# jesselasse/MARL-DMFB

Measured on AMD Instinct MI355X. Metric: env-steps/sec (whole node), 10x10 DMFB 4-droplet fov9, higher is better.
Workload: dtype int8 env state/obs + f64 rewards; fp32 Q-net; 1 GPU; DMFB 10x10, drop_num=4, fov=9, 4096 parallel envs per GPU (BASELINE configs[1]); parallelism=dp1: chips sharded per rank, one flat RCCL all-reduce per learn

## Files before the change

### marl_dmfb_amd/csrc/crnn_ops.hip

```cpp
#include <hip/hip_runtime.h>

#include <cstdint>
#include <cstdio>
#include <cstdlib>

#include "../../include/crnn_ops.h"

#define HIP_ABI_TAG "crnn_ops"
#define HIP_ABI_ERR CRNN_ERR_HIP
#include "hip_abi.h"
#include "crnn_mfma.h"
#include "crnn_mfma19.h"
#include "crnn_bwd19.h"

namespace {

constexpr int kBlock = 512;
constexpr int kA1Stride = 52;
constexpr int kDz1Unit = 108;

constexpr int kLdsBudget = 158 * 1024;

template <int OD> struct GeoB {
    static constexpr int DZ2 = 28;
    static constexpr int DZ_ROW = OD * DZ2 + 4;
    static constexpr int ROW_FLOATS = OD * kA1Stride + OD * DZ2 + 4 + 244 + (OD / 2) * kDz1Unit;
    static constexpr int FIXED_FLOATS = OD * OD * 9;
    static constexpr int RBB = ((kLdsBudget / 4 - FIXED_FLOATS) / ROW_FLOATS) < (kBlock / (2 * OD)) ? ((kLdsBudget / 4 - FIXED_FLOATS) / ROW_FLOATS)
                                                                                                   : (kBlock / (2 * OD));
    static constexpr size_t LDS_FLOATS = (size_t)FIXED_FLOATS + (size_t)RBB * ROW_FLOATS + OD * 28;
    static constexpr int UNITS = OD * (OD / 2);
    static constexpr int NA = UNITS >= kBlock ? kBlock : kBlock / 2;
    static constexpr int NB = UNITS - NA;
    static constexpr int XSLICES = NB > 0 ? (kBlock - NA) / NB : 1;
    static_assert(NB >= 0 && (NB == 0 || (NA + NB * XSLICES <= kBlock && XSLICES <= 8)), "dW2 roles");
    static constexpr int ITEMS3 = (OD / 2) * 9;
    static constexpr int RS3 = kBlock / ITEMS3;
    static constexpr int PART = kBlock * 9 + kBlock * 9 + OD + kBlock * 6 + OD;
};

template <int OD>
__global__ __launch_bounds__(kBlock) void k_conv9_bwd(const int8_t *__restrict__ obs, long obs_stride, long rows,
                                                      const float *__restrict__ a2, long a2_stride, const float *__restrict__ g, long g_stride,
                                                      const float *__restrict__ w2, float *__restrict__ part,
                                                      const float *__restrict__ w1, const float *__restrict__ b1) {
    using G = GeoB<OD>;
    extern __shared__ __attribute__((aligned(16))) float lds[];
    float *s_w2 = lds;
    float *s_a1 = s_w2 + OD * OD * 9;
    float *s_dz2 = s_a1 + G::RBB * OD * kA1Stride;
    float *s_in = s_dz2 + G::RBB * G::DZ_ROW;
    float *s_dz1 = s_in + G::RBB * 244;
    float *s_w1 = s_dz1 + G::RBB * (OD / 2) * kDz1Unit;
    const int tid = threadIdx.x;
    for (int i = tid; i < OD * 27; i += kBlock) s_w1[i] = w1[i];
    if (tid < OD) s_w1[OD * 27 + tid] = b1[tid];
    for (int i = tid; i < OD * OD * 9; i += kBlock) {
        const int c2 = i / (OD * 9), rem = i - c2 * OD * 9, c1 = rem / 9, tap = rem - c1 * 9;
        s_w2[(c2 * 9 + tap) * OD + c1] = w2[i];
    }
    float accB2 = 0.0f, accB1 = 0.0f, accB1y = 0.0f;
    float2 accW2[9], accW1[3];
#pragma unroll
    for (int k = 0; k < 9; ++k) accW2[k] = make_float2(0.0f, 0.0f);
#pragma unroll
    for (int k = 0; k < 3; ++k) accW1[k] = make_float2(0.0f, 0.0f);
    const bool pa_full = tid < G::NA;
    const int pa_unit = pa_full ? tid : G::NA + (G::NB > 0 ? (tid - G::NA) % (G::NB > 0 ? G::NB : 1) : 0);
    const int pa_slice = pa_full ? 0 : (G::NB > 0 ? (tid - G::NA) / (G::NB > 0 ? G::NB : 1) : 0);
    const bool pa_on = pa_full || (G::NB > 0 && pa_slice < G::XSLICES);
    const int pa_step = pa_full ? 1 : G::XSLICES;
    const int pa_c2 = pa_unit / (OD / 2), pa_cp = pa_unit - pa_c2 * (OD / 2);
    const int i3 = tid % G::ITEMS3, s3 = tid / G::ITEMS3;
    const bool p3_on = s3 < G::RS3;
    const int cp_3 = i3 / 9, c0_3 = (i3 - cp_3 * 9) / 3, kx_3 = i3 - cp_3 * 9 - c0_3 * 3;

    constexpr int kSplit2 = G::NB > 0 ? 2 : 4, kBase2 = G::NB > 0 ? kBlock / 2 : 0;
    const int q2 = (tid - kBase2) & (kSplit2 - 1), unit2 = tid >= kBase2 ? (tid - kBase2) / kSplit2 : G::RBB * (OD / 2);
    const int r2 = unit2 / (OD / 2), cp2 = unit2 - r2 * (OD / 2);
    const int br = tid / OD, bc = tid - br * OD;

    const long n_blocks = (rows + G::RBB - 1) / G::RBB;
    const long per = (n_blocks + gridDim.x - 1) / gridDim.x;
    const long blk0 = (long)blockIdx.x * per, blk1 = min(n_blocks, blk0 + per);

    typedef float f32x4 __attribute__((ext_vector_type(4)));
    const int lane = tid & 63, wave = tid >> 6, j16 = lane & 15, kq = lane >> 4;
    const int c_nh = (wave >> 1) & 1, c_sub = (wave & 1) + 2 * (wave >> 2), c_ch = c_nh * 16 + j16;
    const bool c_chv = c_ch < OD;
    constexpr int NPD = (G::RBB * OD * 25 + kBlock - 1) / kBlock, NPI = (G::RBB * 243 + kBlock - 1) / kBlock;
    float pfa[NPD], pfg[NPD];
    int pfi[NPI];
#pragma unroll
    for (int u = 0; u < NPD; ++u) { pfa[u] = 0.0f; pfg[u] = 0.0f; }
#pragma unroll
    for (int u = 0; u < NPI; ++u) pfi[u] = 0;
    auto fetch = [&](long b) {
        const long r0 = b * G::RBB;
        const int rvb = b < blk1 ? (int)min((long)G::RBB, rows - r0) : 0;
        if (rvb <= 0) return;
        int t_ = tid;
        asm volatile("" : "+v"(t_));
#pragma unroll
        for (int u = 0; u < NPD; ++u) {
            const int i = min(t_ + u * kBlock, G::RBB * OD * 25 - 1), rr = i / (OD * 25), rem = i - rr * OD * 25;
            const long row = r0 + min(rr, rvb - 1);
            pfa[u] = a2[row * a2_stride + rem];
            pfg[u] = g[row * g_stride + rem];
        }
#pragma unroll
        for (int u = 0; u < NPI; ++u) {
            const int i = min(t_ + u * kBlock, G::RBB * 243 - 1), rr = i / 243, pp = i - rr * 243;
            pfi[u] = obs[(r0 + min(rr, rvb - 1)) * obs_stride + pp];
        }
    };
    fetch(blk0);
    for (long blk = blk0; blk < blk1; ++blk) {
        const long row0 = blk * G::RBB;
        const int rv = (int)min((long)G::RBB, rows - row0);
        __syncthreads();
        int t_ = tid;
        asm volatile("" : "+v"(t_));
#pragma unroll
        for (int u = 0; u < NPD; ++u) {
            const int i = t_ + u * kBlock, rc = i / 25, k = i - rc * 25;
            if (i < G::RBB * OD * 25) s_dz2[(rc / OD) * G::DZ_ROW + (rc % OD) * G::DZ2 + k] = (rc / OD < rv && pfa[u] > 0.0f) ? pfg[u] : 0.0f;
        }
#pragma unroll
        for (int u = 0; u < NPI; ++u) {
            const int i = t_ + u * kBlock, rr = i / 243, pp = i - rr * 243;
            if (i < G::RBB * 243) s_in[rr * 244 + pp] = rr < rv ? (float)pfi[u] : 0.0f;
        }
        __syncthreads();
        int off1[7], goff[3];
        float bw1[7];
        int kq_ = kq, j_ = j16;
        asm volatile("" : "+v"(kq_), "+v"(j_));
#pragma unroll
        for (int s = 0; s < 7; ++s) {
            const int k = 4 * s + kq_, c0 = k / 9, tap = k - c0 * 9;
            off1[s] = k < 27 ? c0 * 81 + (tap / 3) * 9 + tap % 3 : 0;
            const float w = s_w1[(c_chv ? c_ch : 0) * 27 + (k < 27 ? k : 0)];
            bw1[s] = (c_chv && k < 27) ? w : 0.0f;
        }
        const float c_bias = c_chv ? s_w1[OD * 27 + c_ch] : 0.0f;
#pragma unroll
        for (int qt = 0; qt < 3; ++qt) { const int p = qt * 16 + j_; goff[qt] = (p / 7) * 9 + p % 7; }
        for (int rr = c_sub; rr < G::RBB; rr += 4) {
            float cv[3][7];
#pragma unroll
            for (int qt = 0; qt < 3; ++qt)
#pragma unroll
                for (int s = 0; s < 7; ++s) cv[qt][s] = s_in[rr * 244 + goff[qt] + off1[s]];
            f32x4 acc[3];
#pragma unroll
            for (int qt = 0; qt < 3; ++qt) acc[qt] = f32x4{c_bias, c_bias, c_bias, c_bias};
#pragma unroll
            for (int s = 0; s < 7; ++s)
#pragma unroll
                for (int qt = 0; qt < 3; ++qt) acc[qt] = __builtin_amdgcn_mfma_f32_16x16x4f32(cv[qt][s], bw1[s], acc[qt], 0, 0, 0);
            if (c_chv) {
                float *dst = s_a1 + ((rr * (OD / 2) + (c_ch >> 1)) * kA1Stride + kq * 4) * 2 + (c_ch & 1);
#pragma unroll
                for (int qt = 0; qt < 3; ++qt)
#pragma unroll
                    for (int q = 0; q < 4; ++q) dst[(qt * 16 + q) * 2] = fmaxf(acc[qt][q], 0.0f);
            }
        }
        if (c_sub == 0) {
            const int rr = j16 < G::RBB ? j16 : G::RBB - 1;
            f32x4 acc = {c_bias, c_bias, c_bias, c_bias};
#pragma unroll
            for (int s = 0; s < 7; ++s) acc = __builtin_amdgcn_mfma_f32_16x16x4f32(s_in[rr * 244 + 60 + off1[s]], bw1[s], acc, 0, 0, 0);
            if (c_chv) {
#pragma unroll
                for (int q = 0; q < 4; ++q)
                    if (kq * 4 + q < G::RBB) s_a1[(((kq * 4 + q) * (OD / 2) + (c_ch >> 1)) * kA1Stride + 48) * 2 + (c_ch & 1)] = fmaxf(acc[q], 0.0f);
            }
        }
        __syncthreads();
        auto unit_rows = [&](int c2, int cp, int r_begin, int r_step) {
#pragma unroll 1
            for (int rr = r_begin; rr < rv; rr += r_step) {
                float dz[G::DZ2];
                float2 a[kA1Stride];
                const float4 *pd = (const float4 *)__builtin_assume_aligned(s_dz2 + rr * G::DZ_ROW + c2 * G::DZ2, 16);
                const float4 *pa = (const float4 *)__builtin_assume_aligned(s_a1 + (size_t)(rr * (OD / 2) + cp) * 2 * kA1Stride, 16);
#pragma unroll
                for (int j = 0; j < G::DZ2 / 4; ++j) { const float4 t = pd[j]; dz[4 * j] = t.x; dz[4 * j + 1] = t.y; dz[4 * j + 2] = t.z; dz[4 * j + 3] = t.w; }
#pragma unroll
                for (int j = 0; j < kA1Stride / 2; ++j) { const float4 t = pa[j]; a[2 * j] = make_float2(t.x, t.y); a[2 * j + 1] = make_float2(t.z, t.w); }
#pragma unroll
                for (int kx = 0; kx < 3; ++kx)
#pragma unroll
                    for (int ky = 0; ky < 3; ++ky)
#pragma unroll
                        for (int x = 0; x < 5; ++x)
#pragma unroll
                            for (int y = 0; y < 5; ++y) {
                                const float z = dz[x * 5 + y];
                                const float2 v = a[(x + kx) * 7 + y + ky];
                                accW2[kx * 3 + ky].x = fmaf(z, v.x, accW2[kx * 3 + ky].x);
                                accW2[kx * 3 + ky].y = fmaf(z, v.y, accW2[kx * 3 + ky].y);
                            }
            }
        };
        if (tid < G::RBB * OD && br < rv) {
            const float4 *pd = (const float4 *)__builtin_assume_aligned(s_dz2 + br * G::DZ_ROW + bc * G::DZ2, 16);
            float t = 0.0f;
#pragma unroll
            for (int j = 0; j < 6; ++j) { const float4 v = pd[j]; t += (v.x + v.y) + (v.z + v.w); }
            accB2 += t + pd[6].x;
        }
#ifndef CRNN_PROBE_SKIP_P1
        if (pa_on) unit_rows(pa_c2, pa_cp, pa_slice, pa_step);
#endif
#ifndef CRNN_PROBE_SKIP_P2
        const bool p2 = unit2 < G::RBB * (OD / 2) && r2 < rv;
#else
        const bool p2 = false;
#endif
        if (p2) {
            float2 da[49];
#pragma unroll
            for (int k = 0; k < 49; ++k) da[k] = make_float2(0.0f, 0.0f);
            const int cbeg = q2 * (OD / kSplit2), cend = cbeg + OD / kSplit2;
#pragma unroll 1
            for (int c2 = cbeg; c2 < cend; ++c2) {
                float dz[G::DZ2];
                float2 w[9];
                const float4 *pd = (const float4 *)__builtin_assume_aligned(s_dz2 + r2 * G::DZ_ROW + c2 * G::DZ2, 16);
#pragma unroll
                for (int j = 0; j < G::DZ2 / 4; ++j) { const float4 t = pd[j]; dz[4 * j] = t.x; dz[4 * j + 1] = t.y; dz[4 * j + 2] = t.z; dz[4 * j + 3] = t.w; }
#pragma unroll
                for (int k = 0; k < 9; ++k) w[k] = *(const float2 *)(s_w2 + (c2 * 9 + k) * OD + 2 * cp2);
#pragma unroll
                for (int kx = 0; kx < 3; ++kx)
#pragma unroll
                    for (int ky = 0; ky < 3; ++ky)
#pragma unroll
                        for (int x = 0; x < 5; ++x)
#pragma unroll
                            for (int y = 0; y < 5; ++y) {
                                float2 &d = da[(x + kx) * 7 + y + ky];
                                const float z = dz[x * 5 + y];
                                d.x = fmaf(z, w[kx * 3 + ky].x, d.x);
                                d.y = fmaf(z, w[kx * 3 + ky].y, d.y);
                            }
            }
#ifndef CRNN_PROBE_P2_NO_DPP
#pragma unroll
            for (int k = 0; k < 49; ++k) {
                asm volatile("v_add_f32_dpp %0, %0, %0 quad_perm:[1,0,3,2] row_mask:0xf bank_mask:0xf bound_ctrl:1" : "+v"(da[k].x));
                asm volatile("v_add_f32_dpp %0, %0, %0 quad_perm:[1,0,3,2] row_mask:0xf bank_mask:0xf bound_ctrl:1" : "+v"(da[k].y));
            }
            if (kSplit2 == 4) {
                asm volatile("s_nop 1");
#pragma unroll
                for (int k = 0; k < 49; ++k) {
                    asm volatile("v_add_f32_dpp %0, %0, %0 quad_perm:[2,3,0,1] row_mask:0xf bank_mask:0xf bound_ctrl:1" : "+v"(da[k].x));
                    asm volatile("v_add_f32_dpp %0, %0, %0 quad_perm:[2,3,0,1] row_mask:0xf bank_mask:0xf bound_ctrl:1" : "+v"(da[k].y));
                }
            }
#endif
#ifdef CRNN_PROBE_P2_NO_MASK
            if (q2 == 0 && da[0].x == 12345.678f) {
#else
            if (q2 == 0) {
#endif
                const float4 *act = (const float4 *)__builtin_assume_aligned(s_a1 + (size_t)unit2 * 2 * kA1Stride, 16);
                unsigned long long lx = 0, ly = 0;
#pragma unroll
                for (int j = 0; j < 25; ++j) {
                    const float4 a = act[j];
                    lx |= (unsigned long long)((a.x > 0.0f ? 1u : 0u) | (a.z > 0.0f ? 2u : 0u)) << (2 * j);
                    ly |= (unsigned long long)((a.y > 0.0f ? 1u : 0u) | (a.w > 0.0f ? 2u : 0u)) << (2 * j);
                }
                float4 *dst4 = (float4 *)__builtin_assume_aligned(s_dz1 + (size_t)unit2 * kDz1Unit, 16);
                float sx = 0.0f, sy = 0.0f;
#pragma unroll
                for (int j = 0; j < 25; ++j) {
                    float4 o;
                    o.x = (lx >> (2 * j)) & 1 ? da[2 * j].x : 0.0f;
                    o.y = (ly >> (2 * j)) & 1 ? da[2 * j].y : 0.0f;
                    o.z = (2 * j + 1 < 49 && ((lx >> (2 * j + 1)) & 1)) ? da[2 * j + 1 < 49 ? 2 * j + 1 : 0].x : 0.0f;
                    o.w = (2 * j + 1 < 49 && ((ly >> (2 * j + 1)) & 1)) ? da[2 * j + 1 < 49 ? 2 * j + 1 : 0].y : 0.0f;
                    dst4[j] = o;
                    sx += o.x + o.z;
                    sy += o.y + o.w;
                }
                accB1 += sx;
                accB1y += sy;
            }
        }
        __syncthreads();
        fetch(blk + 1);
#ifdef CRNN_PROBE_SKIP_P3
        if (false) {
#else
        if (p3_on) {
#endif
            for (int rr = s3; rr < rv; rr += G::RS3) {
                const float2 *pd = (const float2 *)(s_dz1 + (size_t)(rr * (OD / 2) + cp_3) * kDz1Unit);
                const float *in = s_in + rr * 244 + c0_3 * 81 + kx_3 * 9;
#pragma unroll
                for (int x = 0; x < 7; ++x) {
                    float2 dz[7];
                    float v[9];
#pragma unroll
                    for (int y = 0; y < 7; ++y) dz[y] = pd[x * 7 + y];
#pragma unroll
                    for (int y = 0; y < 9; ++y) v[y] = in[x * 9 + y];
#pragma unroll
                    for (int ky = 0; ky < 3; ++ky)
#pragma unroll
                        for (int y = 0; y < 7; ++y) {
                            typedef float f32x2 __attribute__((ext_vector_type(2)));
                            const f32x2 r = __builtin_elementwise_fma((f32x2){dz[y].x, dz[y].y}, (f32x2){v[y + ky], v[y + ky]},
                                                                      (f32x2){accW1[ky].x, accW1[ky].y});
                            accW1[ky] = make_float2(r.x, r.y);
                        }
                }
            }
        }
    }
    __syncthreads();
    if (tid < G::RBB * OD) s_dz2[OD * 16 + bc * 16 + br] = accB2;
    if (q2 == 0 && unit2 < G::RBB * (OD / 2)) {
        s_dz2[(2 * cp2) * 16 + r2] = accB1;
        s_dz2[(2 * cp2 + 1) * 16 + r2] = accB1y;
    }
    __syncthreads();
    float *pp = part + (size_t)blockIdx.x * G::PART;
#pragma unroll
    for (int k = 0; k < 9; ++k) { pp[tid * 18 + 2 * k] = accW2[k].x; pp[tid * 18 + 2 * k + 1] = accW2[k].y; }
    if (tid < OD) {
        float t = 0.0f;
        for (int k = 0; k < G::RBB; ++k) t += s_dz2[OD * 16 + tid * 16 + k];
        pp[kBlock * 18 + tid] = t;
    }
#pragma unroll
    for (int k = 0; k < 3; ++k) { pp[kBlock * 18 + OD + tid * 6 + k] = accW1[k].x; pp[kBlock * 18 + OD + tid * 6 + 3 + k] = accW1[k].y; }
    if (tid < OD) {
        float t = 0.0f;
        for (int k = 0; k < G::RBB; ++k) t += s_dz2[tid * 16 + k];
        pp[kBlock * 18 + OD + kBlock * 6 + tid] = t;
    }
}

constexpr int kRedY = 16;
template <int OD>
__global__ __launch_bounds__(64 * kRedY) void k_conv9_bwd_reduce(const float *__restrict__ part, int n_part, float *__restrict__ grads) {
    using G = GeoB<OD>;
    __shared__ float s_sum[kRedY][64];
    const int tx = threadIdx.x & 63, ty = threadIdx.x >> 6;
    const int i = blockIdx.x * 64 + tx;
    const int n2 = OD * OD * 9, nb = OD, n1 = OD * 27;
    float acc = 0.0f;
    if (i < n2 + nb + n1 + nb) {
        int off[8], cnt = 0;
        if (i < n2) {
            const int pair = i / 9, tap = i - pair * 9, c2 = pair / OD, c1 = pair - c2 * OD;
            const int unit = c2 * (OD / 2) + (c1 >> 1), comp = 2 * tap + (c1 & 1);
            if (unit < G::NA) off[cnt++] = unit * 18 + comp;
            else
                for (int sl = 0; sl < G::XSLICES && sl < 8; ++sl) off[cnt++] = (G::NA + sl * G::NB + (unit - G::NA)) * 18 + comp;
        } else if (i < n2 + nb) {
            off[cnt++] = kBlock * 18 + (i - n2);
        } else if (i < n2 + nb + n1) {
            const int jx = i - n2 - nb, c1 = jx / 27, r = jx - c1 * 27, ky = r % 3;
            const int item = (c1 >> 1) * 9 + r / 3;
            for (int sl = 0; sl < G::RS3; ++sl) off[cnt++] = kBlock * 18 + OD + (sl * G::ITEMS3 + item) * 6 + (c1 & 1) * 3 + ky;
        } else {
            off[cnt++] = kBlock * 18 + OD + kBlock * 6 + (i - n2 - nb - n1);
        }
        for (int k = 0; k < cnt; ++k) {
            float a0 = 0.0f, a1 = 0.0f;
            int b = ty;
            for (; b + kRedY < n_part; b += 2 * kRedY) { a0 += part[(size_t)b * G::PART + off[k]]; a1 += part[(size_t)(b + kRedY) * G::PART + off[k]]; }
            if (b < n_part) a0 += part[(size_t)b * G::PART + off[k]];
            acc += a0 + a1;
        }
    }
    s_sum[ty][tx] = acc;
    __syncthreads();
    if (ty == 0 && i < n2 + nb + n1 + nb) {
        float t = 0.0f;
#pragma unroll
        for (int k = 0; k < kRedY; ++k) t += s_sum[k][tx];
        grads[i] = t;
    }
}

constexpr int kMlpBlock = 256, kMlpOut = 10, kMlpMaxIn = 18, kMlpMaxParts = 256, kMlpTailLoads = 64;
__device__ unsigned g_mlp_ticket = 0;
__global__ __launch_bounds__(kMlpBlock) void k_mlp_bwd(const int8_t *__restrict__ obs, long obs_stride, int dir_off,
                                                       const int8_t *__restrict__ onehot, int n_actions, long rows,
                                                       const float *__restrict__ x, long x_stride, const float *__restrict__ g, long g_stride,
                                                       int col0, float *part, float *__restrict__ dw, float *__restrict__ db) {
    __shared__ float s_red[kMlpBlock / 64][kMlpOut * (kMlpMaxIn + 1)];
    __shared__ int s_last;
    const int nin = 2 + n_actions, n_part = (int)gridDim.x;
    float acc[kMlpOut][kMlpMaxIn + 1];
#pragma unroll
    for (int o = 0; o < kMlpOut; ++o)
#pragma unroll
        for (int k = 0; k <= kMlpMaxIn; ++k) acc[o][k] = 0.0f;
    for (long r = (long)blockIdx.x * kMlpBlock + threadIdx.x; r < rows; r += (long)gridDim.x * kMlpBlock) {
        float v[kMlpMaxIn];
        v[0] = (float)obs[r * obs_stride + dir_off];
        v[1] = (float)obs[r * obs_stride + dir_off + 1];
#pragma unroll
        for (int k = 0; k < kMlpMaxIn - 2; ++k) v[2 + k] = k < n_actions ? (float)onehot[r * n_actions + k] : 0.0f;
#pragma unroll
        for (int o = 0; o < kMlpOut; ++o) {
            const float gz = x[r * x_stride + col0 + o] > 0.0f ? g[r * g_stride + col0 + o] : 0.0f;
#pragma unroll
            for (int k = 0; k < kMlpMaxIn; ++k)
                if (k < nin) acc[o][k] = fmaf(gz, v[k], acc[o][k]);
            acc[o][kMlpMaxIn] += gz;
        }
    }
    const int lane = threadIdx.x & 63, wave = threadIdx.x >> 6;
#pragma unroll
    for (int o = 0; o < kMlpOut; ++o)
#pragma unroll
        for (int k = 0; k <= kMlpMaxIn; ++k)
            if (k < nin || k == kMlpMaxIn) {
                float t = acc[o][k];
                for (int d = 32; d > 0; d >>= 1) t += __shfl_xor(t, d);
                if (lane == 0) s_red[wave][o * (kMlpMaxIn + 1) + k] = t;
            }
    __syncthreads();
    const int n_out = kMlpOut * (nin + 1);
    for (int i = threadIdx.x; i < n_out; i += kMlpBlock) {
        const int o = i < kMlpOut * nin ? i / nin : i - kMlpOut * nin, k = i < kMlpOut * nin ? i - o * nin : kMlpMaxIn;
        float t = 0.0f;
#pragma unroll
        for (int w = 0; w < kMlpBlock / 64; ++w) t += s_red[w][o * (kMlpMaxIn + 1) + k];
        part[(size_t)i * n_part + blockIdx.x] = t;
    }
    if (!last_workgroup_arrives(&g_mlp_ticket, gridDim.x, &s_last)) return;
    for (int i = threadIdx.x; i < n_out; i += kMlpBlock) {
        const float *p = part + (size_t)i * n_part;
        float t = 0.0f;
        for (int b0 = 0; b0 < n_part; b0 += kMlpTailLoads) {
            float v[kMlpTailLoads];
#pragma unroll
            for (int u = 0; u < kMlpTailLoads; ++u) v[u] = b0 + u < n_part ? partial_load(p + b0 + u) : 0.0f;
#pragma unroll
            for (int u = 0; u < kMlpTailLoads; ++u)
                if (b0 + u < n_part) t += v[u];
        }
        if (i < kMlpOut * nin) dw[i] = t;
        else db[i - kMlpOut * nin] = t;
    }
}

struct LiveRows { const int32_t *chips; const int32_t *n; int rows_per_chip; };

template <int OD, int RBV>
int launch_rb(const int8_t *obs, long obs_stride, long rows, const float *w1, const float *b1, const float *w2, const float *b2,
              float *out, long out_stride, int out_cols, const int8_t *onehot, int n_actions, const float *mlp_w, const float *mlp_b, hipStream_t s,
              LiveRows live = LiveRows{nullptr, nullptr, 1}) {
    using GM = crnn_mfma::GeoM<OD, RBV>;
    const size_t lds = GM::LDS_FLOATS * sizeof(float);
    static LdsLimit lds_limit;
    if (const int rc = lds_limit.raise((const void *)crnn_mfma::k_conv9_mfma<OD, RBV>, lds)) return rc;
    const long n_blocks = (rows + GM::RB - 1) / GM::RB;
    const long resident = 256L * (long)((size_t)160 * 1024 / lds);
    const int grid = (int)(n_blocks < resident ? n_blocks : resident);
    LAUNCH((crnn_mfma::k_conv9_mfma<OD, RBV>), dim3(grid), dim3(crnn_mfma::kBlockM), lds, s, obs, obs_stride, rows, w1, b1, w2, b2,
           out, out_stride, out_cols, onehot, n_actions, mlp_w, mlp_b, live.chips, live.n, live.rows_per_chip);
    return CRNN_OK;
}

template <int OD>
int launch(const int8_t *obs, long obs_stride, long rows, const float *w1, const float *b1, const float *w2, const float *b2,
           float *out, long out_stride, int out_cols, const int8_t *onehot, int n_actions, const float *mlp_w, const float *mlp_b, hipStream_t s,
           LiveRows live = LiveRows{nullptr, nullptr, 1}) {
    return launch_rb<OD, 0>(obs, obs_stride, rows, w1, b1, w2, b2, out, out_stride, out_cols, onehot, n_actions, mlp_w, mlp_b, s, live);
}

template <int OD>
int launch19(const int8_t *obs, long obs_stride, long rows, const float *w1, const float *b1, const float *w3, const float *b3,
             float *out, long out_stride, int out_cols, const int8_t *onehot, int n_actions, const float *mlp_w, const float *mlp_b, hipStream_t s) {
    using GM = crnn_mfma19::Geo<OD>;
    const size_t lds = GM::LDS_FLOATS * sizeof(float);
    static LdsLimit lds_limit;
    if (const int rc = lds_limit.raise((const void *)crnn_mfma19::k_conv19_mfma<OD>, lds)) return rc;
    const long n_blocks = (rows + GM::RB - 1) / GM::RB;
    const int grid = (int)(n_blocks < 256 ? n_blocks : 256);
    LAUNCH((crnn_mfma19::k_conv19_mfma<OD>), dim3(grid), dim3(crnn_mfma19::kBlockM), lds, s, obs, obs_stride, rows, w1, b1, w3,
           b3, out, out_stride, out_cols, onehot, n_actions, mlp_w, mlp_b);
    return CRNN_OK;
}

template <int OD>
int launch_bwd(const int8_t *obs, long obs_stride, long rows, const float *a2, long a2_stride,
               const float *g, long g_stride, const float *w2, float *part, int grid, float *grads, const float *w1, const float *b1,
               hipStream_t s) {
    using G = GeoB<OD>;
    const size_t lds = G::LDS_FLOATS * sizeof(float);
    static LdsLimit lds_limit;
    if (const int rc = lds_limit.raise((const void *)k_conv9_bwd<OD>, lds)) return rc;
    HIP_TRY(launch_status([&] {
        hipLaunchKernelGGL((k_conv9_bwd<OD>), dim3(grid), dim3(kBlock), lds, s, obs, obs_stride, rows, a2, a2_stride, g, g_stride,
                           w2, part, w1, b1);
        const int n_out = OD * OD * 9 + OD + OD * 27 + OD;
        hipLaunchKernelGGL((k_conv9_bwd_reduce<OD>), dim3((n_out + 63) / 64), dim3(64 * kRedY), 0, s, part, grid, grads);
    }));
    return CRNN_OK;
}

template <int OD>
int launch_bwd19(const int8_t *obs, long obs_stride, long rows, const float *a3, long a3_stride, const float *g, long g_stride,
                 const float *w1, const float *b1, const float *w3, const float *b3, float *part, int n_part, float *grads, hipStream_t s) {
    using G = crnn_bwd19::GeoB19<OD>;
    const size_t lds = G::LDS_FLOATS * sizeof(float);
    static LdsLimit lds_limit;
    if (const int rc = lds_limit.raise((const void *)crnn_bwd19::k_conv19_bwd<OD>, lds)) return rc;
    const long n_blocks = (rows + G::RBB - 1) / G::RBB;
    const int grid = (int)(n_blocks < n_part ? n_blocks : n_part);
    HIP_TRY(launch_status([&] {
        hipLaunchKernelGGL((crnn_bwd19::k_conv19_bwd<OD>), dim3(grid), dim3(crnn_bwd19::kBlockB), lds, s, obs, obs_stride, rows, a3, a3_stride, g,
                           g_stride, w1, b1, w3, b3, part);
        hipLaunchKernelGGL((crnn_bwd19::k_conv19_bwd_reduce<OD>), dim3((G::GRADS + 63) / 64), dim3(64 * crnn_bwd19::kRedY19), 0, s, part, grid, grads);
    }));
    return CRNN_OK;
}

}

// ... 104 lines not shown
```

### marl_dmfb_amd/csrc/crnn_mfma.h

```cpp
#pragma once
#include <hip/hip_runtime.h>

#include <cstdint>

namespace crnn_mfma {

typedef float f32x4 __attribute__((ext_vector_type(4)));

constexpr int kBlockM = 512;

#ifdef CRNN_PROBE_TS
__device__ unsigned long long *g_crnn_ts;
#define CRNN_TS(k) do { if (lane == 0 && ts_it == 1 && g_crnn_ts) g_crnn_ts[((size_t)blockIdx.x * 8 + wave) * 16 + (k)] = __builtin_readcyclecounter(); } while (0)
#else
#define CRNN_TS(k) do { } while (0)
#endif

template <int OD, int RBV = 0, int NW = 8> struct GeoM {
    static constexpr int RB = RBV ? RBV : (OD <= 24 ? 16 : 12);
    static constexpr int CS = 53;
#ifdef CRNN_NO_ROWLANE
    static constexpr bool ROWLANE = false;
#else
    static constexpr bool ROWLANE = RB == 16;
// ... 124 lines not shown
#pragma unroll
        for (int i = 0; i < GS; ++i)
#pragma unroll
            for (int n = 0; n < NT; ++n) {
                const int k = (g % GPQ) * GS + i;
                acc[n] = __builtin_amdgcn_mfma_f32_16x16x4f32(v[g & 1][n][i], bw[(g / GPQ) * 12 + k], acc[n], 0, 0, 0);
            }
        __builtin_amdgcn_sched_barrier(0);
    }
#ifdef CRNN_PROBE_NO_EPI
    if (ok && acc[0][0] == 12345.678f) {
#else
    if (ok) {
#endif
#pragma unroll
        for (int n = 0; n < NT; ++n) {
            float *dst = s_out + kq * 4 * G::OUT_STRIDE + col + (n == 0 ? p0 : p1);
#pragma unroll
            for (int q = 0; q < 4; ++q) dst[q * G::OUT_STRIDE] = fmaxf(acc[n][q], 0.0f);
        }
    }
}

template <int OD, int RBV = 0, int NW = 8>
__global__ __launch_bounds__(64 * NW) void k_conv9_mfma(const int8_t *__restrict__ obs, long obs_stride, long rows,
                                                        const float *__restrict__ w1, const float *__restrict__ b1,
                                                        const float *__restrict__ w2, const float *__restrict__ b2,
                                                        float *__restrict__ out, long out_stride, int out_cols,
                                                        const int8_t *__restrict__ onehot, int n_actions,
                                                        const float *__restrict__ mlp_w, const float *__restrict__ mlp_b,
                                                        const int32_t *__restrict__ live_chips, const int32_t *__restrict__ n_live,
                                                        int rows_per_chip) {
    using G = GeoM<OD, RBV, NW>;
    constexpr int kBlockM = G::BLOCK;
    extern __shared__ __attribute__((aligned(16))) float lds[];
    float *s_in = lds;
    float *s_a1 = s_in + G::RB * G::IN_STRIDE;
    float *s_out = s_a1 + G::RB * G::ROW_A1;
    float *s_vec = s_out + G::RB * G::OUT_STRIDE;
    float *s_mlp = s_vec + G::RB * G::VEC;
    const int tid = threadIdx.x, lane = tid & 63, wave = tid >> 6;
    const int nh = (wave >> 1) & 1, sub = (wave & 1) + 2 * (wave >> 2);
    const int j = lane & 15, kq = lane >> 4;
    const int ch = nh * 16 + j;
    const bool chv = ch < OD;

    if (live_chips) rows = min(rows, (long)n_live[0] * rows_per_chip);
    const long n_blocks = (rows + G::RB - 1) / G::RB;
    const int nin = 2 + n_actions;
    if (mlp_w) {
        for (int i = tid; i < 10 * nin; i += kBlockM) s_mlp[i] = mlp_w[i];
        if (tid < 10) s_mlp[10 * G::VEC + tid] = mlp_b[tid];
    }
    const uint32_t rpc = (uint32_t)(rows_per_chip > 0 ? rows_per_chip : 1);
    const uint32_t rpc_magic = rpc > 1 ? (uint32_t)(0x100000000ull / rpc) + 1u : 0u;
    auto src_row = [&](long cr) -> long {
        if (!live_chips) return cr;
        const uint32_t k = rpc > 1 ? __umulhi((uint32_t)cr, rpc_magic) : (uint32_t)cr;
        return (long)((uint32_t)live_chips[k] * rpc + ((uint32_t)cr - k * rpc));
    };
    constexpr int RPW = (G::RB + NW - 1) / NW, ROWB = 245;
    const int wave_u = __builtin_amdgcn_readfirstlane(wave);
    int pf[RPW][4], pfo[RPW];
    int pf_rv = 0;
#pragma unroll
    for (int h = 0; h < RPW; ++h) {
        pfo[h] = 0;
#pragma unroll
        for (int v = 0; v < 4; ++v) pf[h][v] = 0;
    }
    const int p3 = min(lane + 192, mlp_w ? ROWB - 1 : 242);
    auto fetch = [&](long b) {
        const long r0 = b * G::RB;
        pf_rv = b < n_blocks ? (int)min((long)G::RB, rows - r0) : 0;
#pragma unroll
        for (int h = 0; h < RPW; ++h) {
            const int rr = wave_u + NW * h;
            if (rr < pf_rv) {
                const long sr = src_row(r0 + rr);
                const int8_t *row = obs + sr * obs_stride;
                pf[h][0] = row[lane];
                pf[h][1] = row[lane + 64];
                pf[h][2] = row[lane + 128];
                pf[h][3] = row[p3];
                if (mlp_w && onehot && n_actions > 0) pfo[h] = onehot[sr * n_actions + min(lane, n_actions - 1)];
            }
        }
    };
    auto park = [&]() {
#pragma unroll
        for (int h = 0; h < RPW; ++h) {
            const int rr = wave_u + NW * h;
            if (rr < G::RB) {
                const bool on = rr < pf_rv;
                float *dst = s_in + rr * G::IN_STRIDE;
#pragma unroll
                for (int v = 0; v < 3; ++v) dst[lane + 64 * v] = on ? (float)pf[h][v] : 0.0f;
                const float last = on ? (float)pf[h][3] : 0.0f;
                if (lane + 192 < 243) dst[lane + 192] = last;
                else if (lane + 192 < ROWB) s_vec[rr * G::VEC + lane + 192 - 243] = last;
                if (lane < 16) s_vec[rr * G::VEC + 2 + lane] = (on && onehot && lane < n_actions) ? (float)pfo[h] : 0.0f;
            }
        }
    };
    fetch(blockIdx.x);

    for (int i = tid; i < OD * OD * 9; i += kBlockM) s_a1[i] = w2[i];
    for (int i = tid; i < OD * 27; i += kBlockM) s_in[i] = w1[i];
    __syncthreads();
    float bw1[7];
    int off1[7];
#pragma unroll
    for (int s = 0; s < 7; ++s) {
        const int k = 4 * s + kq;
        const bool kv = k < 27;
        bw1[s] = (chv && kv) ? s_in[ch * 27 + k] : 0.0f;
        const int c0 = k / 9, tap = k - c0 * 9;
        off1[s] = kv ? c0 * 81 + (tap / 3) * 9 + tap % 3 : (G::ROWLANE ? 1 : 0);
    }
    int goff[3];
#pragma unroll
    for (int qt = 0; qt < 3; ++qt) { const int p = qt * 16 + j; goff[qt] = (p / 7) * 9 + p % 7; }
    const int wave_r = __builtin_amdgcn_readfirstlane(wave);
    const int bkind = !G::PAIR || wave_r < 4 ? 0 : wave_r == 5 ? 2 : 1;
    const int xe = j >> 3, bch = G::PAIR ? (bkind == 0 ? j : 16 + (j & 7)) : ch;
    float bw2[G::PAIR ? G::NSTEPX : G::NSTEP2];
    if constexpr (G::PAIR) {
#pragma unroll
        for (int cq = 0; cq < G::KQ; ++cq)
#pragma unroll
            for (int u = 0; u < 12; ++u) {
                const int ty = bkind == 1 ? u / 4 : bkind == 2 ? u / 3 - xe : u / 3;
                const int tx = bkind == 1 ? u % 4 - xe : u % 3;
                const bool ok = ty >= 0 && ty < 3 && tx >= 0 && tx < 3;
                bw2[cq * 12 + u] = ok ? s_a1[(bch * OD + 4 * cq + kq) * 9 + ty * 3 + tx] : 0.0f;
            }
    } else {
#pragma unroll
        for (int cq = 0; cq < G::KQ; ++cq)
#pragma unroll
            for (int tap = 0; tap < 9; ++tap) bw2[cq * 9 + tap] = chv ? s_a1[(ch * OD + 4 * cq + kq) * 9 + tap] : 0.0f;
    }
    __syncthreads();
    const float bias1 = chv ? b1[ch] : 0.0f, bias2 = G::PAIR ? b2[bch] : chv ? b2[ch] : 0.0f;
    const int n_feat = OD * 25 + (mlp_w ? 10 : 0);
    const int n_out = out_cols > n_feat ? out_cols : n_feat;
    const bool wide_out = (out_stride % 2 == 0) && (((size_t)out) % 8 == 0) && (n_out % 2 == 0);
    const bool quad_out = (out_stride % 4 == 0) && (((size_t)out) % 16 == 0) && (n_out % 4 == 0) && (G::OUT_STRIDE % 4 == 0);
    for (int i = tid; i < G::RB * (G::OUT_STRIDE - n_feat); i += kBlockM) {
        const int rr = i / (G::OUT_STRIDE - n_feat), k = i - rr * (G::OUT_STRIDE - n_feat);
        s_out[rr * G::OUT_STRIDE + n_feat + k] = 0.0f;
    }

    park();
    __syncthreads();
#ifdef CRNN_PROBE_TS
    int ts_it = 0;
#endif
    for (long blk = blockIdx.x; blk < n_blocks; blk += gridDim.x) {
        CRNN_TS(0);
        const long row0 = blk * G::RB;
        const int rv = (int)min((long)G::RB, rows - row0);
        float mv = 0.0f;
        const int mr = tid / 10, mc = tid - mr * 10;
        if (mlp_w && tid < G::RB * 10) {
            mv = s_mlp[10 * G::VEC + mc];
            for (int k = 0; k < nin; ++k) mv = fmaf(s_vec[mr * G::VEC + k], s_mlp[mc * nin + k], mv);
        }
        fetch(blk + gridDim.x);
        CRNN_TS(1);
#ifndef CRNN_PROBE_SKIP_CONV1
        if constexpr (G::ROWLANE) {
            constexpr int NT1 = 49, NIT = (NT1 / G::NSUB) / 3;
            static_assert(G::NSUB == 4 && NIT * 3 * G::NSUB == NT1 - 1, "conv1 row-lane tiling");
            const int sub_u = __builtin_amdgcn_readfirstlane(sub);
            int jb = j * G::IN_STRIDE;
            asm volatile("" : "+v"(jb));
            int lb[7];
#pragma unroll
            for (int s = 0; s < 7; ++s) lb[s] = jb + off1[s];
            auto spos = [&](int m) {
                const int p = sub_u + G::NSUB * m;
                return (p / 7) * 9 + p % 7;
            };
            float cv[2][3][7];
#pragma unroll
            for (int c = 0; c < 3; ++c) {
                const int sp = spos(c);
#pragma unroll
                for (int s = 0; s < 7; ++s) cv[0][c][s] = s_in[lb[s] + sp];
            }
#pragma unroll
            for (int it = 0; it < NIT; ++it) {
                if (it + 1 < NIT) {
#pragma unroll
                    for (int c = 0; c < 3; ++c) {
                        const int sp = spos(3 * (it + 1) + c);
#pragma unroll
                        for (int s = 0; s < 7; ++s) cv[(it + 1) & 1][c][s] = s_in[lb[s] + sp];
                    }
                } else if (sub_u == 0) {
#pragma unroll
                    for (int s = 0; s < 7; ++s) cv[(it + 1) & 1][0][s] = s_in[lb[s] + 60];
                }
                __builtin_amdgcn_sched_barrier(0);
                f32x4 acc[3];
#pragma unroll
                for (int c = 0; c < 3; ++c) acc[c] = f32x4{bias1, bias1, bias1, bias1};
#pragma unroll
                for (int s = 0; s < 7; ++s)
#pragma unroll
                    for (int c = 0; c < 3; ++c) acc[c] = __builtin_amdgcn_mfma_f32_16x16x4f32(cv[it & 1][c][s], bw1[s], acc[c], 0, 0, 0);
                __builtin_amdgcn_sched_barrier(0);
                if (chv) {
#pragma unroll
                    for (int c = 0; c < 3; ++c) {
                        float *dst = s_a1 + kq * 4 * G::ROW_A1 + ch * G::CS + sub_u + G::NSUB * (3 * it + c);
#pragma unroll
                        for (int q = 0; q < 4; ++q) dst[q * G::ROW_A1] = fmaxf(acc[c][q], 0.0f);
                    }
                }
            }
            if (sub_u == 0) {
                f32x4 acc = {bias1, bias1, bias1, bias1};
#pragma unroll
                for (int s = 0; s < 7; ++s) acc = __builtin_amdgcn_mfma_f32_16x16x4f32(cv[NIT & 1][0][s], bw1[s], acc, 0, 0, 0);
                if (chv) {
                    float *dst = s_a1 + kq * 4 * G::ROW_A1 + ch * G::CS + 48;
#pragma unroll
                    for (int q = 0; q < 4; ++q) dst[q * G::ROW_A1] = fmaxf(acc[q], 0.0f);
                }
            }
        } else {
            int gq[3];
#pragma unroll
            for (int qt = 0; qt < 3; ++qt) { gq[qt] = goff[qt] + sub * G::IN_STRIDE; asm volatile("" : "+v"(gq[qt])); }
            float cv[2][3][7];
#pragma unroll
            for (int qt = 0; qt < 3; ++qt)
#pragma unroll
                for (int s = 0; s < 7; ++s) cv[0][qt][s] = s_in[gq[qt] + off1[s]];
#pragma unroll
            for (int i = 0; i < G::RB / G::NSUB; ++i) {
                if (i + 1 < G::RB / G::NSUB) {
#pragma unroll
                    for (int qt = 0; qt < 3; ++qt)
#pragma unroll
                        for (int s = 0; s < 7; ++s)
                            cv[(i + 1) & 1][qt][s] = s_in[G::NSUB * (i + 1) * G::IN_STRIDE + gq[qt] + off1[s]];
                }
                __builtin_amdgcn_sched_barrier(0);
                f32x4 acc[3];
#pragma unroll
                for (int qt = 0; qt < 3; ++qt) acc[qt] = f32x4{bias1, bias1, bias1, bias1};
#pragma unroll
                for (int s = 0; s < 7; ++s)
#pragma unroll
                    for (int qt = 0; qt < 3; ++qt) acc[qt] = __builtin_amdgcn_mfma_f32_16x16x4f32(cv[i & 1][qt][s], bw1[s], acc[qt], 0, 0, 0);
                __builtin_amdgcn_sched_barrier(0);
                if (chv) {
                    float *dst = s_a1 + (sub + G::NSUB * i) * G::ROW_A1 + ch * G::CS + kq * 4;
#pragma unroll
                    for (int qt = 0; qt < 3; ++qt)
#pragma unroll
                        for (int q = 0; q < 4; ++q) dst[qt * 16 + q] = fmaxf(acc[qt][q], 0.0f);
                }
            }
            if (sub == 0) {
                const int rr = j < G::RB ? j : G::RB - 1;
                f32x4 acc = {bias1, bias1, bias1, bias1};
#pragma unroll
                for (int s = 0; s < 7; ++s) acc = __builtin_amdgcn_mfma_f32_16x16x4f32(s_in[rr * G::IN_STRIDE + 60 + off1[s]], bw1[s], acc, 0, 0, 0);
                if (chv) {
#pragma unroll
                    for (int q = 0; q < 4; ++q)
                        if (kq * 4 + q < G::RB) s_a1[(kq * 4 + q) * G::ROW_A1 + ch * G::CS + 48] = fmaxf(acc[q], 0.0f);
                }
            }
        }
#endif
        CRNN_TS(2);
        __syncthreads();
        CRNN_TS(3);
        park();
        CRNN_TS(4);
#ifndef CRNN_PROBE_SKIP_CONV2
        if constexpr (G::PAIR) {
            const int col = bch * 25 + (bkind == 1 ? xe : bkind == 2 ? 5 * xe : 0);
            constexpr int T9 = 0, PH = 1, PV = 2;
            if (wave_r < 4) {
                const int pa = wave_r < 2 ? 7 * wave_r : wave_r == 2 ? 14 : 20;
                conv2_rl_tiles<OD, 2, T9>(s_a1, s_out, bw2, bias2, pa, pa + 1, col, true, j, kq);
                conv2_rl_tiles<OD, 2, T9>(s_a1, s_out, bw2, bias2, pa + 2, pa + 3, col, true, j, kq);
                if (wave_r < 3) conv2_rl_tiles<OD, 2, T9>(s_a1, s_out, bw2, bias2, pa + 4, pa + 5, col, true, j, kq);
                if (wave_r != 2) { const int pl = wave_r == 3 ? 24 : pa + 6; conv2_rl_tiles<OD, 1, T9>(s_a1, s_out, bw2, bias2, pl, pl, col, true, j, kq); }
            } else if (wave_r == 5) {
                conv2_rl_tiles<OD, 2, PV>(s_a1, s_out, bw2, bias2, 4, 14, col, true, j, kq);
                conv2_rl_tiles<OD, 1, PV>(s_a1, s_out, bw2, bias2, 19, 19, col, xe == 1, j, kq);
            } else {
                const int q0 = wave_r == 4 ? 0 : wave_r == 6 ? 3 : 6;
                auto pos = [](int q) { return (q >> 1) * 5 + (q & 1) * 2; };
                conv2_rl_tiles<OD, 2, PH>(s_a1, s_out, bw2, bias2, pos(q0), pos(q0 + 1), col, true, j, kq);
                if (wave_r == 7) conv2_rl_tiles<OD, 2, PH>(s_a1, s_out, bw2, bias2, pos(q0 + 2), pos(q0 + 3), col, true, j, kq);
                else conv2_rl_tiles<OD, 1, PH>(s_a1, s_out, bw2, bias2, pos(q0 + 2), pos(q0 + 2), col, true, j, kq);
            }
        } else {
            int t = sub;
#ifdef CRNN_PROBE_TS
            int ts_k = 8;
#endif
#pragma unroll 1
            for (; t + G::NSUB < G::T2; t += 2 * G::NSUB) {
                conv2_tiles<OD, RBV, 2>(s_a1, s_out, bw2, bias2, t, t + G::NSUB, j, kq, ch, chv);
#ifdef CRNN_PROBE_TS
                CRNN_TS(ts_k); ++ts_k;
#endif
            }
            if (t < G::T2) conv2_tiles<OD, RBV, 1>(s_a1, s_out, bw2, bias2, t, t, j, kq, ch, chv);
        }
#endif
        if (mlp_w && tid < G::RB * 10) s_out[mr * G::OUT_STRIDE + OD * 25 + mc] = fmaxf(mv, 0.0f);
        CRNN_TS(5);
        __syncthreads();
        CRNN_TS(6);
#ifndef CRNN_PROBE_SKIP_OUT
        if (quad_out) {
            for (int rr = wave; rr < rv; rr += kBlockM / 64) {
                float4 *dst = (float4 *)(out + (row0 + rr) * out_stride);
                const float4 *src = (const float4 *)(s_out + rr * G::OUT_STRIDE);
                for (int k = lane; k < n_out / 4; k += 64) dst[k] = src[k];
            }
        } else if (wide_out) {
            for (int rr = wave; rr < rv; rr += kBlockM / 64) {
                float2 *dst = (float2 *)(out + (row0 + rr) * out_stride);
                const float2 *src = (const float2 *)(s_out + rr * G::OUT_STRIDE);
                for (int k = lane; k < n_out / 2; k += 64) dst[k] = src[k];
            }
        } else {
            for (int rr = wave; rr < rv; rr += kBlockM / 64) {
                float *dst = out + (row0 + rr) * out_stride;
                const float *src = s_out + rr * G::OUT_STRIDE;
                for (int k = lane; k < n_out; k += 64) dst[k] = src[k];
            }
        }
#endif
        CRNN_TS(7);
#ifdef CRNN_PROBE_TS
        ++ts_it;
#endif
    }
}


}
```

Before: 7.764 million env-steps/s.

## Split dz1 ReLU-mask stage across two lanes and unroll bwd-reduce partial loads

The dz1 masking step in the conv9 backward kernel now runs on two lanes per unit (one for x, one for y channel) using scalar LDS reads, where before one lane did both with float4 loads. The a1 row stride shrinks from 52 to 50 floats, which changes LDS footprint and may raise rows per block. The reduce kernel issues all partial loads into registers up front (fixed 8x2 unroll, which assumes at most 256 partials) so more loads are in flight. The prefetch also zeroes its registers on empty blocks. The trade-off is lost float4 vectorization and possible new LDS bank conflicts.

```diff
diff --git a/marl_dmfb_amd/csrc/crnn_ops.hip b/marl_dmfb_amd/csrc/crnn_ops.hip
--- a/marl_dmfb_amd/csrc/crnn_ops.hip
+++ b/marl_dmfb_amd/csrc/crnn_ops.hip
@@ -16,7 +16,7 @@
 namespace {
 
 constexpr int kBlock = 512;
-constexpr int kA1Stride = 52;
+constexpr int kA1Stride = 50;
 constexpr int kDz1Unit = 108;
 
 constexpr int kLdsBudget = 158 * 1024;
@@ -59,7 +59,7 @@
         const int c2 = i / (OD * 9), rem = i - c2 * OD * 9, c1 = rem / 9, tap = rem - c1 * 9;
         s_w2[(c2 * 9 + tap) * OD + c1] = w2[i];
     }
-    float accB2 = 0.0f, accB1 = 0.0f, accB1y = 0.0f;
+    float accB2 = 0.0f, accB1 = 0.0f;
     float2 accW2[9], accW1[3];
 #pragma unroll
     for (int k = 0; k < 9; ++k) accW2[k] = make_float2(0.0f, 0.0f);
@@ -98,7 +98,13 @@
     auto fetch = [&](long b) {
         const long r0 = b * G::RBB;
         const int rvb = b < blk1 ? (int)min((long)G::RBB, rows - r0) : 0;
-        if (rvb <= 0) return;
+        if (rvb <= 0) {
+#pragma unroll
+            for (int u = 0; u < NPD; ++u) { pfa[u] = 0.0f; pfg[u] = 0.0f; }
+#pragma unroll
+            for (int u = 0; u < NPI; ++u) pfi[u] = 0;
+            return;
+        }
         int t_ = tid;
         asm volatile("" : "+v"(t_));
 #pragma unroll
@@ -264,33 +270,25 @@
             }
 #endif
 #ifdef CRNN_PROBE_P2_NO_MASK
-            if (q2 == 0 && da[0].x == 12345.678f) {
+            if (q2 < 2 && da[0].x == 12345.678f) {
 #else
-            if (q2 == 0) {
+            if (q2 < 2) {
 #endif
-                const float4 *act = (const float4 *)__builtin_assume_aligned(s_a1 + (size_t)unit2 * 2 * kA1Stride, 16);
-                unsigned long long lx = 0, ly = 0;
+                const float *act = s_a1 + (size_t)unit2 * 2 * kA1Stride + q2;
+                float *dst = s_dz1 + (size_t)unit2 * kDz1Unit + q2;
+                const bool odd = q2 != 0;
+                float sb = 0.0f;
 #pragma unroll
                 for (int j = 0; j < 25; ++j) {
-                    const float4 a = act[j];
-                    lx |= (unsigned long long)((a.x > 0.0f ? 1u : 0u) | (a.z > 0.0f ? 2u : 0u)) << (2 * j);
-                    ly |= (unsigned long long)((a.y > 0.0f ? 1u : 0u) | (a.w > 0.0f ? 2u : 0u)) << (2 * j);
+                    const float2 d0 = da[2 * j], d1 = da[2 * j + 1 < 49 ? 2 * j + 1 : 0];
+                    const float v0 = odd ? d0.y : d0.x, v1 = odd ? d1.y : d1.x;
+                    const float o0 = act[4 * j] > 0.0f ? v0 : 0.0f;
+                    const float o1 = (2 * j + 1 < 49 && act[2 * j + 1 < 49 ? 4 * j + 2 : 0] > 0.0f) ? v1 : 0.0f;
+                    dst[4 * j] = o0;
+                    dst[4 * j + 2] = o1;
+                    sb += o0 + o1;
                 }
-                float4 *dst4 = (float4 *)__builtin_assume_aligned(s_dz1 + (size_t)unit2 * kDz1Unit, 16);
-                float sx = 0.0f, sy = 0.0f;
-#pragma unroll
-                for (int j = 0; j < 25; ++j) {
-                    float4 o;
-                    o.x = (lx >> (2 * j)) & 1 ? da[2 * j].x : 0.0f;
-                    o.y = (ly >> (2 * j)) & 1 ? da[2 * j].y : 0.0f;
-                    o.z = (2 * j + 1 < 49 && ((lx >> (2 * j + 1)) & 1)) ? da[2 * j + 1 < 49 ? 2 * j + 1 : 0].x : 0.0f;
-                    o.w = (2 * j + 1 < 49 && ((ly >> (2 * j + 1)) & 1)) ? da[2 * j + 1 < 49 ? 2 * j + 1 : 0].y : 0.0f;
-                    dst4[j] = o;
-                    sx += o.x + o.z;
-                    sy += o.y + o.w;
-                }
-                accB1 += sx;
-                accB1y += sy;
+                accB1 += sb;
             }
         }
         __syncthreads();
@@ -326,10 +324,7 @@
     }
     __syncthreads();
     if (tid < G::RBB * OD) s_dz2[OD * 16 + bc * 16 + br] = accB2;
-    if (q2 == 0 && unit2 < G::RBB * (OD / 2)) {
-        s_dz2[(2 * cp2) * 16 + r2] = accB1;
-        s_dz2[(2 * cp2 + 1) * 16 + r2] = accB1y;
-    }
+    if (q2 < 2 && unit2 < G::RBB * (OD / 2)) s_dz2[(2 * cp2 + q2) * 16 + r2] = accB1;
     __syncthreads();
     float *pp = part + (size_t)blockIdx.x * G::PART;
 #pragma unroll
@@ -349,6 +344,7 @@
 }
 
 constexpr int kRedY = 16;
+static_assert(2 * kRedY * 8 >= 256, "k_conv9_bwd_reduce holds the <= 256 partial vectors of an output as 2 x 8 loads per thread");
 template <int OD>
 __global__ __launch_bounds__(64 * kRedY) void k_conv9_bwd_reduce(const float *__restrict__ part, int n_part, float *__restrict__ grads) {
     using G = GeoB<OD>;
@@ -375,10 +371,19 @@
             off[cnt++] = kBlock * 18 + OD + kBlock * 6 + (i - n2 - nb - n1);
         }
         for (int k = 0; k < cnt; ++k) {
+            float v0[8], v1[8];
+#pragma unroll
+            for (int m = 0; m < 8; ++m) {
+                const int b0 = ty + 2 * kRedY * m, b1 = b0 + kRedY;
+                v0[m] = b0 < n_part ? part[(size_t)b0 * G::PART + off[k]] : 0.0f;
+                v1[m] = b1 < n_part ? part[(size_t)b1 * G::PART + off[k]] : 0.0f;
+            }
             float a0 = 0.0f, a1 = 0.0f;
-            int b = ty;
-            for (; b + kRedY < n_part; b += 2 * kRedY) { a0 += part[(size_t)b * G::PART + off[k]]; a1 += part[(size_t)(b + kRedY) * G::PART + off[k]]; }
-            if (b < n_part) a0 += part[(size_t)b * G::PART + off[k]];
+#pragma unroll
+            for (int m = 0; m < 8; ++m) {
+                if (ty + 2 * kRedY * m < n_part) a0 += v0[m];
+                if (ty + 2 * kRedY * m + kRedY < n_part) a1 += v1[m];
+            }
             acc += a0 + a1;
         }
     }
```

After: 7.790 million env-steps/s (median of 2 runs). About the same (+0.3%).

## Defer CRNN output tile store to overlap with next block's conv1

Applied to the files above, without the earlier changes.

On the row-lane, 8-wave path with float4-aligned output, the per-block copy of s_out to global memory is no longer done right after the barrier. Waves 0-3 now store the previous block's rows at the start of the next iteration, alongside conv1, and a final flush after the loop writes the last block. This aims to hide the global store latency behind conv1 compute and remove a serialized phase from each iteration. In exchange it relies on s_out staying untouched until conv2 rewrites it, and it puts the store work unevenly on half the waves.

```diff
diff --git a/marl_dmfb_amd/csrc/crnn_mfma.h b/marl_dmfb_amd/csrc/crnn_mfma.h
--- a/marl_dmfb_amd/csrc/crnn_mfma.h
+++ b/marl_dmfb_amd/csrc/crnn_mfma.h
@@ -300,6 +300,27 @@
         s_out[rr * G::OUT_STRIDE + n_feat + k] = 0.0f;
     }
 
+    constexpr bool DEFER = G::ROWLANE && NW == 8;
+    const bool defer = DEFER && quad_out;
+    long d_row0 = 0;
+    int d_rv = 0;
+    const int n4 = n_out / 4;
+    auto stream_rows = [&](int step, int first) {
+#pragma unroll
+        for (int h = 0; h < 4; ++h) {
+            const int rr = first + step * h;
+            if (rr < d_rv) {
+                const float4 *src = (const float4 *)(s_out + rr * G::OUT_STRIDE);
+                float4 *dst = (float4 *)(out + (d_row0 + rr) * out_stride);
+                const float4 v0 = src[lane], v1 = src[lane + 64], v2 = src[min(lane + 128, G::OUT_STRIDE / 4 - 1)];
+#ifndef CRNN_PROBE_SKIP_OUT
+                if (lane < n4) dst[lane] = v0;
+                if (lane + 64 < n4) dst[lane + 64] = v1;
+                if (lane + 128 < n4) dst[lane + 128] = v2;
+#endif
+            }
+        }
+    };
     park();
     __syncthreads();
 #ifdef CRNN_PROBE_TS
@@ -317,6 +338,9 @@
         }
         fetch(blk + gridDim.x);
         CRNN_TS(1);
+        if constexpr (DEFER) {
+            if (defer && wave_r < 4) stream_rows(4, wave_u);
+        }
 #ifndef CRNN_PROBE_SKIP_CONV1
         if constexpr (G::ROWLANE) {
             constexpr int NT1 = 49, NIT = (NT1 / G::NSUB) / 3;
@@ -472,7 +496,10 @@
         __syncthreads();
         CRNN_TS(6);
 #ifndef CRNN_PROBE_SKIP_OUT
-        if (quad_out) {
+        if (defer) {
+            d_row0 = row0;
+            d_rv = rv;
+        } else if (quad_out) {
             for (int rr = wave; rr < rv; rr += kBlockM / 64) {
                 float4 *dst = (float4 *)(out + (row0 + rr) * out_stride);
                 const float4 *src = (const float4 *)(s_out + rr * G::OUT_STRIDE);
@@ -497,6 +524,9 @@
         ++ts_it;
 #endif
     }
+    if constexpr (DEFER) {
+        if (defer) stream_rows(8, wave_u);
+    }
 }
 
 
```

New measurement: 7.735 million env-steps/s before, 7.744 million env-steps/s after, median of 2. No clear change (+0.1%).
